# YoungWook0533/dyros_robot_controller

Hardware: AMD Instinct MI355X
Metric: QP-IK solves/s (FR3 7-DoF, batch 65k) + achieved HBM GB/s vs peak (higher is better)
Workload: dtype f64; 1 GPU; FR3 QPIKStep (exact: certified OSQP polish), 65536 instances per GPU; robot=fr3, batch_per_gpu=65536, global_batch=65536, solver=exact, parallelism=dp1 (instances sharded, no data-path collective), task_stage=wave-per-instance

## Files before the change

### dyros_robot_controller_amd/csrc/api.cpp

```cpp
#include <hip/hip_runtime.h>

#include <chrono>
#include <cmath>
#include <cstdlib>
#include <cstddef>
#include <cstdio>
#include <cstring>
#include <memory>
#include <mutex>
#include <string>
#include <algorithm>
#include <vector>

#include "../../include/drc_amd.h"
#include "../../include/drc_amd_debug.h"
#include "dynamics.hpp"
#include "kernel_common.hpp"
#include "launch.hpp"
#include "mesh.hpp"

namespace drc_amd {

struct StreamCtx {
  hipStream_t stream = nullptr;
  hipEvent_t done = nullptr;
  uint64_t last_use = 0;
  void* pool = nullptr;
  int64_t pool_bytes = 0;
  static constexpr int kSlotInts = 32;
  static constexpr int kQueueSlotQpid = 16, kQueueSlotCf = 17, kQueueInts = 18 * kSlotInts;
  int* d_queue = nullptr;
  int* dyn_list = nullptr;
  int64_t dyn_list_cap = 0;
  void* roll = nullptr;
  int64_t roll_bytes = 0;
};
constexpr size_t kMaxStreamCtx = 8;

struct Lanes {
  std::vector<hipStream_t> lanes;
  std::vector<hipEvent_t> joins;
  std::vector<hipStream_t> sides;
  std::vector<hipEvent_t> side_fork, side_join;
  hipEvent_t fork = nullptr;
};

struct drc_model_impl {
  HostModel hm;
  DevModel* d_model = nullptr;
  double* d_mesh = nullptr;
  int device = 0;
  drc_kinematic_param kparam{};
  drc_joint_index jidx{};
  drc_actuator_index aidx{};
  std::vector<std::unique_ptr<StreamCtx>> ctxs;
  uint64_t ctx_tick = 0;
  Lanes ln;
  int timing = 0;
  int lane_stage = 0;
  int eqp_small_cap = -1;
  std::vector<std::pair<std::vector<hipEvent_t>, int>> events;
  std::vector<hipEvent_t> evpool;
  int chunks = 4;
  int fused = 1;
  int32_t* d_order = nullptr;
  int64_t order_n = 0;
  std::mutex host_mu;
  void* stage = nullptr;
  int64_t stage_bytes = 0;
  double* pinned = nullptr;
  int64_t pinned_bytes = 0;
  hipStream_t hstream = nullptr;
  hipEvent_t hdone = nullptr;
  int tl_on = 0;
  std::vector<int64_t> tl;
  std::mutex mu;
  std::mutex launch_mu;
};

static thread_local std::string g_last_error;
static int set_err(int code, const std::string& msg) {
  g_last_error = msg;
  return code;
}
#define HIP_TRY(expr)                                                                   \
  do {                                                                                  \
    hipError_t e_ = (expr);                                                             \
    if (e_ != hipSuccess) return set_err(DRC_ERR_HIP, std::string(#expr) + ": " + hipGetErrorString(e_)); \
  } while (0)

static void free_ctx(StreamCtx* c) {
  if (c->done) (void)hipEventSynchronize(c->done), (void)hipEventDestroy(c->done);
  c->done = nullptr;
  if (c->d_queue) (void)hipFree(c->d_queue);
  if (c->pool) (void)hipFree(c->pool);
  if (c->dyn_list) (void)hipFree(c->dyn_list);
  if (c->roll) (void)hipFree(c->roll);
  c->roll = nullptr;
  c->roll_bytes = 0;
  c->d_queue = nullptr;
  c->pool = nullptr;
  c->dyn_list = nullptr;
}
// ... 163 lines not shown
  const double r = p.wheel_radius;
  if (p.type == DRC_DRIVE_DIFFERENTIAL) {
    *W = 2;
    const double e[6] = {1 / r, 0, -p.base_width / (2 * r), 1 / r, 0, p.base_width / (2 * r)};
    for (int i = 0; i < 6; ++i) J[i] = e[i];
    return DRC_OK;
  }
  if (p.type == DRC_DRIVE_MECANUM) {
    const int n = p.n_wheels;
    if (n < 1 || n > kMaxWheels) return set_err(DRC_ERR_INVALID_ARGUMENT, "mecanum wheel count out of range");
    for (int i = 0; i < n; ++i) {
      const double g = p.roller_angles[i], px = p.base2wheel_positions[i][0], py = p.base2wheel_positions[i][1],
                   pt = p.base2wheel_angles[i];
      const double a0 = std::cos(pt) - std::tan(g) * std::sin(pt), a1 = std::sin(pt) + std::tan(g) * std::cos(pt);
      J[i * 3 + 0] = a0 / r;
      J[i * 3 + 1] = a1 / r;
      J[i * 3 + 2] = (-a0 * py + a1 * px) / r;
    }
    *W = n;
    return DRC_OK;
  }
  if (p.type == DRC_DRIVE_CASTER) {
    const int C = p.n_wheels;
    if (C < 1 || 2 * C > kMaxWheels) return set_err(DRC_ERR_INVALID_ARGUMENT, "caster count out of range");
    const double b = p.wheel_offset;
    for (int i = 0; i < C; ++i) {
      const double phi = wheel_pos ? wheel_pos[2 * i] : 0.0, sp = std::sin(phi), cp = std::cos(phi);
      const double px = p.base2wheel_positions[i][0], py = p.base2wheel_positions[i][1];
      double* r0 = J + (2 * i) * 3;
      double* r1 = J + (2 * i + 1) * 3;
      r0[0] = -sp / b;
      r0[1] = cp / b;
      r0[2] = (px * cp + py * sp) / b - 1;
      r1[0] = cp / r;
      r1[1] = sp / r;
      r1[2] = (px * sp - py * cp) / r;
    }
    *W = 2 * C;
    return DRC_OK;
  }
  return set_err(DRC_ERR_INVALID_ARGUMENT, "unknown drive type");
}

static const char kMeshStageMsg[] =
    "the model has collision meshes: the lane-per-instance debug stage handles sphere, cylinder and box geometry only";

static int upload(drc_model_impl* m) {
  HIP_TRY(hipSetDevice(m->device));
  if (m->hm.has_mesh()) {
    const size_t bytes = m->hm.mesh_verts.size() * sizeof(double);
    HIP_TRY(hipMalloc(&m->d_mesh, bytes));
    HIP_TRY(hipMemcpy(m->d_mesh, m->hm.mesh_verts.data(), bytes, hipMemcpyHostToDevice));
    m->hm.dev.mesh_verts = m->d_mesh;
  }
  HIP_TRY(hipMalloc(&m->d_model, sizeof(DevModel)));
  HIP_TRY(hipMemcpy(m->d_model, &m->hm.dev, sizeof(DevModel), hipMemcpyHostToDevice));
  return DRC_OK;
}

static int plan_layout(const DevModel& M, KParams* k, bool task_only) {
  int off = 0;
  auto take = [&](int n) {
    int o = off;
    off += (n + 1) & ~1;
    return o;
  };
  const int nx = k->nx, ng = k->ng, np = k->np, m = k->m, nv = M.nv;
  if (task_only) {
    k->oRed = take(64);
    k->oSc = take(32);
  } else {
  k->oP = take(np * np);
  k->oG = take(ng * nx);
  k->oQ = take(nx);
  k->oAB = take(nx);
  k->oL = take(m);
  k->oU = take(m);
  k->oD = take(nx);
  k->oE = take(m);
  k->oDi = take(nx);
  k->oEi = take(m);
  k->oRho = take(m);
  k->oX = take(nx);
  k->oZ = take(m);
  k->oY = take(m);
  k->oDY = take(m);
  k->oXT = take(nx);
  k->oZT = take(m);
  k->oT1 = take(m > nx ? m : nx);
  k->oT2 = take(m > nx ? m : nx);
  k->oRed = take(64);
  k->oSc = take(32);
  k->oBc = take(nx + ng > 32 ? nx + ng : 32);
  }
  k->oHi = -1;
  if (!task_only && k->problem == 0 && M.kind == 1 && qp_compiled(nx, ng, np)) k->oHi = take(nx * nx);
  k->oU0 = off;
  if (!task_only && k->problem == 0) {
    int u = k->oU0;
    auto takeu = [&](int n) {
      int o = u;
      u += (n + 1) & ~1;
      return o;
    };
    k->kq = takeu(nv);
    k->kJ = takeu(6 * nv);
// ... 876 lines not shown
  const int virtual_dof = 3;
  d.kind = 1;
  d.n_wheel = W;
  d.n_arm = d.nv - (virtual_dof + W);
  d.virtual_start = ji->virtual_start;
  d.mani_start = ji->mani_start;
  d.mobi_start = ji->mobi_start;
  d.act_mani_start = ai->mani_start;
  d.act_mobi_start = ai->mobi_start;
  d.dyn_origin = ji->virtual_start + 3;
  if (d.n_arm < 1 || d.n_arm > 8 || ji->virtual_start + 3 > d.nv || ji->mani_start + d.n_arm > d.nv ||
      ji->mobi_start + W > d.nv || ai->mani_start + d.n_arm > d.n_arm + W || ai->mobi_start + W > d.n_arm + W) {
    delete m;
    return drc_amd::set_err(DRC_ERR_INVALID_ARGUMENT, "JointIndex/ActuatorIndex inconsistent with the URDF dof");
  }
  m->kparam = *param;
  m->jidx = *ji;
  m->aidx = *ai;
  m->device = device;
  rc = drc_amd::upload(m);
  if (rc) {
    delete m;
    return rc;
  }
  *out = m;
  return DRC_OK;
}

int drc_model_release_stream(drc_model* m, void* stream) {
  using drc_amd::set_err;
  if (!m) return drc_amd::set_err(DRC_ERR_INVALID_ARGUMENT, "null model");
  std::lock_guard<std::mutex> launch_lock(m->launch_mu);
  std::lock_guard<std::mutex> g(m->mu);
  HIP_TRY(hipSetDevice(m->device));
  hipStream_t st = reinterpret_cast<hipStream_t>(stream);
  for (size_t i = 0; i < m->ctxs.size(); ++i)
    if (m->ctxs[i]->stream == st) {
      HIP_TRY(hipStreamSynchronize(st));
      drc_amd::free_ctx(m->ctxs[i].get());
      m->ctxs.erase(m->ctxs.begin() + static_cast<std::ptrdiff_t>(i));
      break;
    }
  return DRC_OK;
}

void drc_model_destroy(drc_model* m) {
  if (!m) return;
  (void)hipSetDevice(m->device);
  (void)hipDeviceSynchronize();
  for (auto& c : m->ctxs) drc_amd::free_ctx(c.get());
  drc_amd::free_lanes(&m->ln);
  if (m->d_model) (void)hipFree(m->d_model);
  if (m->d_mesh) (void)hipFree(m->d_mesh);
  if (m->d_order) (void)hipFree(m->d_order);
  if (m->hstream) (void)hipStreamSynchronize(m->hstream), (void)hipStreamDestroy(m->hstream);
  if (m->stage) (void)hipFree(m->stage);
  if (m->pinned) (void)hipHostFree(m->pinned);
  if (m->hdone) (void)hipEventDestroy(m->hdone);
  for (auto& evs : m->events) {
    std::vector<hipEvent_t> u = evs.first;
    std::sort(u.begin(), u.end());
    u.erase(std::unique(u.begin(), u.end()), u.end());
    for (hipEvent_t e : u) (void)hipEventDestroy(e);
  }
  for (hipEvent_t e : m->evpool) (void)hipEventDestroy(e);
  delete m;
}

int drc_model_info(const drc_model* m, int* dof, int* act, int* mani, int* mobi, int* ngeom, int* npairs) {
  if (!m) return drc_amd::set_err(DRC_ERR_INVALID_ARGUMENT, "null model");
  const drc_amd::DevModel& d = m->hm.dev;
  if (dof) *dof = d.nv;
  if (act) *act = d.kind == 1 ? d.n_arm + d.n_wheel : d.nv;
  if (mani) *mani = d.kind == 1 ? d.n_arm : d.nv;
  if (mobi) *mobi = d.kind == 1 ? d.n_wheel : 0;
  if (ngeom) *ngeom = d.ngeom;
  if (npairs) *npairs = d.npairs;
  return DRC_OK;
}

int drc_model_geom_info(const drc_model* m, int geom, int* type, double param[3], int* n_vertices,
                        double* hull_residual) {
  if (!m) return drc_amd::set_err(DRC_ERR_INVALID_ARGUMENT, "null model");
  const drc_amd::DevModel& d = m->hm.dev;
  if (geom < 0 || geom >= d.ngeom) return drc_amd::set_err(DRC_ERR_INVALID_ARGUMENT, "geometry index out of range");
  if (type) *type = d.gtype[geom];
  if (param)
    for (int i = 0; i < 3; ++i) param[i] = d.gparam[geom][i];
  if (n_vertices) *n_vertices = m->hm.mesh_count[geom];
  if (hull_residual) *hull_residual = m->hm.mesh_residual[geom];
  return DRC_OK;
}

int drc_mesh_convex_hull(const char* path, const double scale[3], int max_vertices, double* verts_out, int cap,
                         int* n_out, double* residual_out) {
  if (!path || !n_out) return drc_amd::set_err(DRC_ERR_INVALID_ARGUMENT, "null argument");
  *n_out = 0;
  drc_amd::MeshHull hull;
  std::string err;
  const int rc = drc_amd::mesh_convex_hull(path, scale, max_vertices > 0 ? max_vertices : drc_amd::kMaxMeshVerts,
                                           &hull, &err);
  if (rc) return drc_amd::set_err(rc, err);
  const int n = static_cast<int>(hull.verts.size());
  *n_out = n;
  if (residual_out) *residual_out = hull.residual;
  if (n > cap || (n > 0 && !verts_out))
// ... 728 lines not shown
```

### dyros_robot_controller_amd/csrc/model.cpp

```cpp
#include "model.hpp"

#include <algorithm>
#include <cmath>
#include <cstdio>
#include <cstring>
#include <fstream>
#include <map>
#include <memory>
#include <set>
#include <sstream>

#include "../../include/drc_amd.h"
#include "mesh.hpp"

namespace drc_amd {
namespace {

struct XmlNode {
  std::string tag;
  std::map<std::string, std::string> attr;
  std::vector<std::unique_ptr<XmlNode>> kids;
  const XmlNode* child(const char* t) const {
    for (auto& k : kids)
      if (k->tag == t) return k.get();
// ... 434 lines not shown
        *err = "SRDF: " + e2;
        return DRC_ERR_PARSE;
      }
      std::set<std::pair<int, int>> drop;
      for (const XmlNode* d : sr->children("disable_collisions")) {
        const char* l1 = d->get("link1");
        const char* l2 = d->get("link2");
        if (!l1 || !l2 || !b.frame_of_link.count(l1) || !b.frame_of_link.count(l2)) continue;
        if (std::string(l1) == l2) continue;
        for (int a = 0; a < m.ngeom; ++a) {
          if (b.geom_link[a] != l1) continue;
          for (int c = 0; c < m.ngeom; ++c)
            if (b.geom_link[c] == l2) drop.insert({std::min(a, c), std::max(a, c)});
        }
      }
      std::vector<std::pair<int, int>> kept;
      for (auto& p : pairs)
        if (!drop.count(p)) kept.push_back(p);
      pairs.swap(kept);
    }
  }
  if (static_cast<int>(pairs.size()) > kMaxPairs) {
    *err = "too many collision pairs";
    return DRC_ERR_UNSUPPORTED;
  }
  m.npairs = static_cast<int>(pairs.size());
  for (int p = 0; p < m.npairs; ++p) {
    m.pair_a[p] = static_cast<int16_t>(pairs[p].first);
    m.pair_b[p] = static_cast<int16_t>(pairs[p].second);
  }
  {
    int n = 0;
    for (int cls = 0; cls < 7; ++cls)
      for (int p = 0; p < m.npairs; ++p) {
        int ta = m.gtype[m.pair_a[p]], tb = m.gtype[m.pair_b[p]];
        if (ta > tb) std::swap(ta, tb);
        const int c = tb == kMesh ? 6 : (ta == 0 ? tb : (ta == 1 ? 2 + tb : 5));
        if (c == cls) m.pair_order[n++] = static_cast<int16_t>(p);
      }
    for (int sl = 0; sl < m.npairs; ++sl) {
      m.slot_a[sl] = m.pair_a[m.pair_order[sl]];
      m.slot_b[sl] = m.pair_b[m.pair_order[sl]];
    }
  }
  m.ncand_slots = 0;
  for (int p = 0; p < m.npairs; ++p) {
    m.cand_slot[p] = -1;
    if (m.gtype[m.pair_a[p]] != kSphere && m.gtype[m.pair_b[p]] != kSphere) {
      if (m.ncand_slots < kMaxCandSlots) m.cand_pair[m.ncand_slots] = static_cast<int16_t>(p);
      m.cand_slot[p] = static_cast<int16_t>(m.ncand_slots < kMaxCandSlots ? m.ncand_slots : -1);
      ++m.ncand_slots;
    }
  }
  return DRC_OK;
}

}
```

### dyros_robot_controller_amd/csrc/model.hpp

```cpp
#pragma once

#include <cstdint>
#include <string>
#include <vector>

namespace drc_amd {

constexpr int kMaxJoints = 16;
constexpr int kMaxGeoms = 64;
constexpr int kMaxPairs = 1024;
constexpr int kMaxFrames = 64;
constexpr int kMaxWheels = 8;
constexpr int kMaxCandSlots = 128;

enum JointType : int { kRevolute = 0, kPrismatic = 1 };
enum GeomType : int { kSphere = 0, kCylinder = 1, kBox = 2, kMesh = 3 };
enum DriveKind : int { kDriveDifferential = 0, kDriveMecanum = 1, kDriveCaster = 2 };

struct DevModel {
  int nv, ngeom, npairs, nframes;
  int kind;
  int n_arm, n_wheel;
  int virtual_start, mani_start, mobi_start;
  int act_mani_start, act_mobi_start;
  int parent[kMaxJoints + 1];
  int jtype[kMaxJoints + 1];
  uint32_t anc[kMaxJoints + 1];
  double jplace[kMaxJoints + 1][12];
  double axis[kMaxJoints + 1][3];
  double lower[kMaxJoints], upper[kMaxJoints], vel[kMaxJoints];
  int frame_joint[kMaxFrames];
  double frame_place[kMaxFrames][12];
  int gparent[kMaxGeoms];
  int gtype[kMaxGeoms];
  double gplace[kMaxGeoms][12];
  double gparam[kMaxGeoms][3];
  double gbound[kMaxGeoms];
  int16_t pair_a[kMaxPairs], pair_b[kMaxPairs];
  int16_t cand_slot[kMaxPairs];
  int16_t cand_pair[kMaxCandSlots];
  int ncand_slots;
  int16_t pair_order[kMaxPairs];
  int16_t slot_a[kMaxPairs], slot_b[kMaxPairs];
  double J_mobile[3][kMaxWheels];
  int drive;
  double wheel_radius, wheel_offset;
  double caster_pos[kMaxWheels / 2][2];
  double inertia[kMaxJoints + 1][10];
  int dyn_origin;
  int has_mesh;
  int gmesh_first[kMaxGeoms], gmesh_count[kMaxGeoms];
  const double* mesh_verts;
};

struct HostModel {
  DevModel dev{};
  std::vector<std::string> joint_names;
  std::vector<std::string> frame_names;
  std::vector<std::string> geom_names;
  std::vector<double> effort;
  std::vector<double> mesh_verts;
  std::vector<int> mesh_first, mesh_count;
  std::vector<double> mesh_residual;
  std::vector<std::string> mesh_files;
  bool has_mesh() const { return !mesh_verts.empty(); }
};

int build_model_from_urdf(const std::string& urdf_path, const std::string& srdf_path,
                          const std::string& packages_path, HostModel* out, std::string* err);

}
```

### dyros_robot_controller_amd/csrc/task_stage.hpp

```cpp
#pragma once

#include "kernel_common.hpp"

namespace drc_amd {

__device__ __forceinline__ void col_dot(const DevModel* M, const double* T, const double* Zw, const double* qd, int nv,
                                        int c, V3 p, V3 pdot, uint32_t mask, V3* lin, V3* ang) {
  const V3 oc = v3(T[12 * c + 9], T[12 * c + 10], T[12 * c + 11]), zc = ld3(Zw + 3 * c);
  V3 w = v3(0, 0, 0), od = v3(0, 0, 0);
  const uint32_t ac = M->anc[c] & mask;
  for (int a = 1; a <= nv; ++a) {
    if (!(ac & (1u << (a - 1)))) continue;
    const V3 za = ld3(Zw + 3 * a);
    if (M->jtype[a] == kRevolute) {
      if (a != c) w = w + qd[a - 1] * za;
      od = od + qd[a - 1] * cross(za, oc - v3(T[12 * a + 9], T[12 * a + 10], T[12 * a + 11]));
    } else {
      od = od + qd[a - 1] * za;
    }
  }
  const V3 zd = cross(w, zc);
  if (M->jtype[c] == kRevolute) {
    *lin = cross(zd, p - oc) + cross(zc, pdot - od);
    *ang = zd;
// ... 256 lines not shown
      for (int c = 0; c < nv; ++c) s += J[l * nv + c] * nu[c];
      vec[l] = xdd[l] - s;
    }
    wsync();
    if (l < nv) {
      double s = nu[l];
      for (int i = 0; i < 6; ++i) s += W[i * nv + l] * vec[i];
      out = s;
    }
  } else {
    for (int e = l; e < 6 * nv; e += 64) {
      const int i = e / nv, c = e % nv;
      double s = 0;
      for (int a = 0; a < nv; ++a) s += J[i * nv + a] * Mi[a * nv + c];
      W[e] = s;
    }
    wsync();
    if (l < 36) {
      const int a = l / 6, b = l % 6;
      double s = 0;
      for (int c = 0; c < nv; ++c) s += W[a * nv + c] * J[b * nv + c];
      A6[l] = s;
    }
    wsync();
    if (!inv6_certified(A6, Ai)) pinv_cod6_wave(A6, Ai, ws);
    for (int e = l; e < 6 * nv; e += 64) {
      const int i = e / nv, c = e % nv;
      double s = 0;
      for (int j = 0; j < 6; ++j) s += Ai[i * 6 + j] * W[j * nv + c];
      W2[e] = s;
    }
    if (l < 6) {
      double s = 0;
      for (int j = 0; j < 6; ++j) s += Ai[l * 6 + j] * xdd[j];
      vec[l] = s;
    }
    wsync();
    if (l < 6) {
      double s = 0;
      for (int c = 0; c < nv; ++c) s += W2[l * nv + c] * nu[c];
      vec[6 + l] = vec[l] - s;
    }
    wsync();
    if (l < nv) {
      double s = gv[l] + nu[l];
      for (int i = 0; i < 6; ++i) s += J[i * nv + l] * vec[6 + i];
      out = s;
    }
  }
  if (l < nv) io.out[(int64_t)l * LD + gb] = out;
  wsync();
}

template <int PROBLEM, bool MESH = false>
__device__ __forceinline__ void task_instance(const DevModel* __restrict__ M0, const KParams& kp, const IO& io, double* S,
                                              int64_t b) {
  const int l = lane_id();
  const int nv = kp.nv;
  EpaPoly* ews = reinterpret_cast<EpaPoly*>(S + kp.kEpa);
  PH_DECL
  const int64_t gb = io.b0 + b, LD = io.ld;
  PH_ONLY(const unsigned long long inst_t0 = __builtin_amdgcn_s_memtime(); unsigned long long ph_snap[8];
          for (int k_ = 0; k_ < 8; ++k_) ph_snap[k_] = ph_acc[k_];
          unsigned long long epa_calls = 0, epa_steps = 0, epa_maxsteps = 0, epa_t[8] = {0, 0, 0, 0, 0, 0, 0, 0};)
  const DevModel* M = opaque_model(M0);
  double* qv = S + kp.kq;
  double* qd = S + kp.kqd;
  if (l < nv) {
    qv[l] = io.q[l * LD + gb];
    qd[l] = io.qdot[l * LD + gb];
  }
  double tgt = 0.0;
  if (PROBLEM == 2 && kp.cf == 3) {
  } else if (l < 12) {
    if (kp.mode != DRC_MODE_QPIK) tgt = io.xt[l * LD + gb];
  } else if (l < 18) {
    tgt = io.xdt[(l - 12) * LD + gb];
  } else if (l < 36 && kp.mode == DRC_MODE_QPIK_CUBIC) {
    tgt = l < 30 ? io.xi[(l - 18) * LD + gb] : io.xdi[(l - 30) * LD + gb];
  }
  wsync();
  double* T = S + kp.kT;
  double* Zw = S + kp.kZ;
  if (l < 12) T[l] = (l == 0 || l == 4 || l == 8) ? 1.0 : 0.0;
  double* loc = S + kp.kTg;
  if (l >= 1 && l <= nv) {
    const int j = l;
    double Mj[12];
    const double* ax = M->axis[j];
    const double qq = qv[j - 1];
    if (M->jtype[j] == kRevolute) {
      double c = cos(qq), s = sin(qq), C = 1 - c, x = ax[0], y = ax[1], z = ax[2];
      Mj[0] = c + x * x * C; Mj[1] = x * y * C - z * s; Mj[2] = x * z * C + y * s;
      Mj[3] = y * x * C + z * s; Mj[4] = c + y * y * C; Mj[5] = y * z * C - x * s;
      Mj[6] = z * x * C - y * s; Mj[7] = z * y * C + x * s; Mj[8] = c + z * z * C;
      Mj[9] = Mj[10] = Mj[11] = 0;
    } else {
      Mj[0] = Mj[4] = Mj[8] = 1;
      Mj[1] = Mj[2] = Mj[3] = Mj[5] = Mj[6] = Mj[7] = 0;
      Mj[9] = ax[0] * qq; Mj[10] = ax[1] * qq; Mj[11] = ax[2] * qq;
    }
    double Lj[12];
    tmul(M->jplace[j], Mj, Lj);
    for (int i = 0; i < 12; ++i) loc[(j - 1) * 12 + i] = Lj[i];
  }
  wsync();
  for (int j = 1; j <= nv; ++j) {
    const double* a = T + M->parent[j] * 12;
    const double* bb = loc + (j - 1) * 12;
    double v = 0;
    if (l < 9) {
      int r = l / 3, c = l % 3;
      v = a[3 * r] * bb[c] + a[3 * r + 1] * bb[3 + c] + a[3 * r + 2] * bb[6 + c];
    } else if (l < 12) {
      int r = l - 9;
      v = a[3 * r] * bb[9] + a[3 * r + 1] * bb[10] + a[3 * r + 2] * bb[11] + a[9 + r];
    }
    wsync();
    if (l < 12) T[j * 12 + l] = v;
    wsync();
  }
  double* Te = S + kp.kTe;
  if (l >= 1 && l <= nv) st3(Zw + 3 * l, rot(T + 12 * l, ld3(M->axis[l])));
  if (l == 0) tmul(T + 12 * kp.frame_joint, kp.frame_place, Te);
  wsync();
  double* Tg = S + kp.kTg;
  for (int g = l; g < M->ngeom; g += 64) {
    double out[12];
    tmul(T + 12 * M->gparent[g], M->gplace[g], out);
    for (int i = 0; i < 12; ++i) Tg[g * 12 + i] = out[i];
  }
  PH(0);
  double* J = S + kp.kJ;
  const V3 pe = v3(Te[9], Te[10], Te[11]);
  const uint32_t anc_e = M->anc[kp.frame_joint];
  if (l < nv) {
    const int j = l + 1;
    V3 lin = v3(0, 0, 0), ang = v3(0, 0, 0);
    if (anc_e & (1u << l)) {
      V3 z = ld3(Zw + 3 * j);
      if (M->jtype[j] == kRevolute) {
        lin = cross(z, pe - v3(T[12 * j + 9], T[12 * j + 10], T[12 * j + 11]));
        ang = z;
      } else {
        lin = z;
      }
    }
    J[0 * nv + l] = lin.x; J[1 * nv + l] = lin.y; J[2 * nv + l] = lin.z;
    J[3 * nv + l] = ang.x; J[4 * nv + l] = ang.y; J[5 * nv + l] = ang.z;
  }
  wsync();
  double* xdd = S + kp.kxdd;
  double jq = 0.0;
  if (l < 6)
    for (int c = 0; c < nv; ++c) jq += J[l * nv + c] * qd[c];
  if (l == 0) {
    if (kp.mode == DRC_MODE_QPIK) {
      for (int i = 0; i < 6; ++i) xdd[i] = rd_lane(tgt, 12 + i);
    } else {
      double xt[12], xdt[6];
      for (int i = 0; i < 12; ++i) xt[i] = rd_lane(tgt, i);
      for (int i = 0; i < 6; ++i) xdt[i] = rd_lane(tgt, 12 + i);
      if (kp.mode == DRC_MODE_QPIK_CUBIC) {
        double xi[12], xdi[6], Rt[9], Ri[9];
        for (int i = 0; i < 12; ++i) xi[i] = rd_lane(tgt, 18 + i);
        for (int i = 0; i < 6; ++i) xdi[i] = rd_lane(tgt, 30 + i);
        for (int r = 0; r < 3; ++r)
          for (int c = 0; c < 3; ++c) {
            Rt[3 * r + c] = xt[3 * c + r];
            Ri[3 * r + c] = xi[3 * c + r];
          }
        const double t = kp.t, t0 = kp.t0, tf = kp.t0 + kp.duration;
        double pd[3], vd[3];
        for (int i = 0; i < 3; ++i) {
          pd[i] = cubic(t, t0, tf, xi[9 + i], xt[9 + i], xdi[i], xdt[i]);
          vd[i] = cubic_dot(t, t0, tf, xi[9 + i], xt[9 + i], xdi[i], xdt[i]);
        }
        double RiT_Rt[9], Rd[9];
        for (int a = 0; a < 3; ++a)
          for (int c = 0; c < 3; ++c)
            RiT_Rt[3 * a + c] = Ri[a] * Rt[c] + Ri[3 + a] * Rt[3 + c] + Ri[6 + a] * Rt[6 + c];
        V3 r = so3_log(RiT_Rt);
        if (t >= tf) {
          for (int i = 0; i < 9; ++i) Rd[i] = Rt[i];
        } else if (t < t0) {
          for (int i = 0; i < 9; ++i) Rd[i] = Ri[i];
        } else {
          double E3[9];
          so3_exp(cubic(t, t0, tf, 0, 1, 0, 0) * r, E3);
          for (int a = 0; a < 3; ++a)
            for (int c = 0; c < 3; ++c)
              Rd[3 * a + c] = Ri[3 * a] * E3[c] + Ri[3 * a + 1] * E3[3 + c] + Ri[3 * a + 2] * E3[6 + c];
        }
        V3 rd = v3(cubic_dot(t, t0, tf, 0, r.x, 0, 0), cubic_dot(t, t0, tf, 0, r.y, 0, 0),
// ... 42 lines not shown
    int a = l / 6, bb = l % 6;
    double s = 0;
    for (int c = 0; c < narm; ++c) s += J[a * nv + c0 + c] * J[bb * nv + c0 + c];
    A6[l] = s;
  }
  wsync();
  {
    double piv_min = 1e300, det = 1;
    const int lr = l < 6 ? l : 0;
    double r6[6];
#pragma unroll
    for (int j = 0; j < 6; ++j) r6[j] = A6[lr * 6 + j];
#pragma unroll
    for (int k = 0; k < 6; ++k) {
      const double akk = bcast(r6[k], k), aik = r6[k], ia = 1.0 / akk;
      double pk6[6];
#pragma unroll
      for (int j = 0; j < 6; ++j) pk6[j] = bcast(r6[j], k);
#pragma unroll
      for (int j = 0; j < 6; ++j) {
        double v;
        if (l == k && j == k) v = ia;
        else if (l == k) v = pk6[j] * ia;
        else if (j == k) v = -aik * ia;
        else v = r6[j] - aik * (pk6[j] * ia);
        r6[j] = v;
      }
      piv_min = fmin(piv_min, akk);
      det *= akk;
    }
    if (l < 6)
#pragma unroll
      for (int j = 0; j < 6; ++j) Ai[l * 6 + j] = r6[j];
    wsync();
    const double fa = wave_sum(l < 36 ? A6[l] * A6[l] : 0.0), fi = wave_sum(l < 36 ? Ai[l] * Ai[l] : 0.0);
    if (!(piv_min > 0) || !(fa * fi < 1e10)) {
      const double dt = det_lu6_wave(A6);
      pinv_cod6_wave(A6, Ai, S + kp.kScr);
      if (l == 0) S[kp.oSc + SC_MAN] = sqrt(dt);
    } else if (l == 0) {
      S[kp.oSc + SC_MAN] = sqrt(det);
    }
    wsync();
  }
  double* W = S + kp.kW;
  for (int e = l; e < narm * 6; e += 64) {
    int c = e / 6, a = e % 6;
    double s = 0;
    for (int i = 0; i < 6; ++i) s += J[i * nv + c0 + c] * Ai[i * 6 + a];
    W[e] = s;
  }
  wsync();
  double* part = S + kp.kPart;
  for (int e = l; e < narm * narm; e += 64) {
    const int kk = e / narm, c = e % narm;
    const int jk = c0 + kk + 1, ji = c0 + c + 1;
    double acc = 0;
    if ((anc_e & (1u << (jk - 1))) && (anc_e & (1u << (ji - 1)))) {
      V3 zk = ld3(Zw + 3 * jk), zi = ld3(Zw + 3 * ji);
      V3 pk_ = v3(T[12 * jk + 9], T[12 * jk + 10], T[12 * jk + 11]);
      V3 pi_ = v3(T[12 * ji + 9], T[12 * ji + 10], T[12 * ji + 11]);
      const bool krev = M->jtype[jk] == kRevolute;
      V3 dpe = krev ? cross(zk, pe - pk_) : zk;
      const bool moves_i = jk != ji && (M->anc[ji] & (1u << (jk - 1)));
      V3 dzi = (moves_i && krev) ? cross(zk, zi) : v3(0, 0, 0);
      V3 dpi = moves_i ? (krev ? cross(zk, pi_ - pk_) : zk) : v3(0, 0, 0);
      V3 lin, ang;
      if (M->jtype[ji] == kRevolute) {
        lin = cross(dzi, pe - pi_) + cross(zi, dpe - dpi);
        ang = dzi;
      } else {
        lin = dzi;
        ang = v3(0, 0, 0);
      }
      const double* w = W + c * 6;
      acc = lin.x * w[0] + lin.y * w[1] + lin.z * w[2] + ang.x * w[3] + ang.y * w[4] + ang.z * w[5];
    }
    part[e] = acc;
  }
  wsync();
  double* mg = S + kp.kmg;
  if (l < narm) {
    double s = 0;
    for (int c = 0; c < narm; ++c) s += part[l * narm + c];
    mg[l] = S[kp.oSc + SC_MAN] * s;
  }
  PH(2);
  double* pd = S + kp.kPd;
  int8_t* pf = reinterpret_cast<int8_t*>(S + kp.kPf);
  double bestd = 1.7976931348623157e308;
  int besti = 0x7fffffff;
  int bhow = 0;
  V3 bpA = v3(0, 0, 0), bpB = v3(0, 0, 0);
  double ub = 1e300;
  [[maybe_unused]] auto hull_shape = [&](int g) {
    return ShapeMT<lds_pose*, true>{M->gtype[g], (lds_pose*)(Tg + 12 * g), M->gparam[g][0], M->gparam[g][1],
                                    M->gparam[g][2], M->mesh_verts + 3 * M->gmesh_first[g], M->gmesh_count[g]};
  };
  for (int sl = l; sl < M->npairs; sl += 64) {
    const int p = M->pair_order[sl], ga = M->slot_a[sl], gb = M->slot_b[sl];
    ShapeL A{M->gtype[ga], (lds_pose*)(Tg + 12 * ga), M->gparam[ga][0], M->gparam[ga][1], M->gparam[ga][2]};
    ShapeL Bs{M->gtype[gb], (lds_pose*)(Tg + 12 * gb), M->gparam[gb][0], M->gparam[gb][1], M->gparam[gb][2]};
    V3 pA, pB;
    double d;
    if constexpr (MESH) {
      if (A.type == kMesh || Bs.type == kMesh) {
        if (A.type == kMesh) A.type = kBox;
        if (Bs.type == kMesh) Bs.type = kBox;
        pd[p] = (A.type == kSphere || Bs.type == kSphere) ? sphere_pair(A, Bs, &pA, &pB)
                                                          : pair_lower_bound(A, Bs, M->gbound[ga], M->gbound[gb]);
        pf[p] = 0;
        continue;
      }
    }
    const bool closed = (A.type == kSphere || Bs.type == kSphere)
                            ? (d = sphere_pair(A, Bs, &pA, &pB), true)
                            : (A.type == kCylinder && Bs.type == kCylinder && cyl_cyl_side(A, Bs, &d, &pA, &pB));
    if (closed) {
      pf[p] = 1;
      ub = fmin(ub, d);
      if (d < bestd || (d == bestd && p < besti)) {
        bestd = d;
        besti = p;
        bhow = 0;
        bpA = pA;
        bpB = pB;
      }
    } else {
      pd[p] = pair_lower_bound(A, Bs, M->gbound[ga], M->gbound[gb]);
      pf[p] = 0;
    }
  }
  ub = -wave_max(-ub);
  PH(3);
  bool pen = false;
  {
    int* cand = reinterpret_cast<int*>(S + kp.kCand);
    int ncand = 0;
    [[maybe_unused]] int nhull = 0;
    for (int p0 = 0; p0 < M->npairs; p0 += 64) {
      const int p = p0 + l;
      bool c = p < M->npairs && pf[p] == 0 && pd[p] - 1e-9 <= ub;
      if constexpr (MESH) {
        const bool h = c && (M->gtype[M->pair_a[p]] == kMesh || M->gtype[M->pair_b[p]] == kMesh);
        const unsigned long long mh = __ballot(h);
        if (h) cand[M->npairs - 1 - (nhull + __popcll(mh & ((1ull << l) - 1)))] = p;
        nhull += __popcll(mh);
        c = c && !h;
      }
      const unsigned long long m = __ballot(c);
      if (c) cand[ncand + __popcll(m & ((1ull << l) - 1))] = p;
      ncand += __popcll(m);
    }
    if (l == 0) ews->nv = 0;
    wsync();
    for (int c = l; c < ncand; c += 64) {
      const int p = cand[c];
      const int ga = M->pair_a[p], gb = M->pair_b[p];
      ShapeL A{M->gtype[ga], (lds_pose*)(Tg + 12 * ga), M->gparam[ga][0], M->gparam[ga][1], M->gparam[ga][2]};
      ShapeL Bs{M->gtype[gb], (lds_pose*)(Tg + 12 * gb), M->gparam[gb][0], M->gparam[gb][1], M->gparam[gb][2]};
      const GjkDist g = gjk(A, Bs, ub + 1e-9, ews, p);
      if (g.pruned) {
        pf[p] = 1;
      } else if (g.intersect) {
        pf[p] = 2;
        pen = true;
      } else {
        pf[p] = 1;
        if (g.dist < bestd || (g.dist == bestd && p < besti)) {
          bestd = g.dist;
          besti = p;
          bhow = 1;
          bpA = g.pA;
          bpB = g.pB;
        }
      }
    }
    if constexpr (MESH) {
      ub = fmin(ub, -wave_max(-bestd));
      for (int c = 0; c < nhull; ++c) {
        const int p = cand[M->npairs - 1 - c];
        const int ga = M->pair_a[p], gb = M->pair_b[p];
// ... 81 lines not shown
        bpB = ld3(ews->out + 3);
      }
      if (dall < gbd || (dall == gbd && p < gbi)) {
        gbd = dall;
        gbi = p;
      }
      if (l == ln) pf[p] = 1;
      wsync();
    }
#ifdef DRC_EPA_PRIO
    __builtin_amdgcn_s_setprio(0);
#endif
  }
  PH(5);
  const double myd = bestd;
  const int myi = besti;
  wave_argmin(bestd, besti);
  double* dgv = S + kp.kdg;
  double* red = S + kp.oRed;
  auto refine_winner = [&]() {
    const int ga = M->pair_a[besti], gb = M->pair_b[besti];
    const ShapeL A{M->gtype[ga], (lds_pose*)(Tg + 12 * ga), M->gparam[ga][0], M->gparam[ga][1], M->gparam[ga][2]};
    const ShapeL Bs{M->gtype[gb], (lds_pose*)(Tg + 12 * gb), M->gparam[gb][0], M->gparam[gb][1], M->gparam[gb][2]};
    double dref = S[kp.oSc + SC_DIST];
    V3 rA = ld3(red), rB = ld3(red + 3);
    if constexpr (MESH) {
      if (A.type == kMesh || Bs.type == kMesh) {
        if (refine_witness_hull(serial_shape(hull_shape(ga)), serial_shape(hull_shape(gb)), &dref, &rA, &rB)) {
          st3(red, rA);
          st3(red + 3, rB);
          S[kp.oSc + SC_DIST] = dref;
        }
        return;
      }
    }
#ifdef DRC_NO_REFINE
    if (false && refine_witness(A, Bs, &dref, &rA, &rB)) {
#else
    if (refine_witness(A, Bs, &dref, &rA, &rB)) {
#endif
      st3(red, rA);
      st3(red + 3, rB);
      S[kp.oSc + SC_DIST] = dref;
    }
  };
  auto dist_grad = [&](double dd) {
    double g = 0;
    if (besti < M->npairs) {
      const int jA = M->gparent[M->pair_a[besti]], jB = M->gparent[M->pair_b[besti]];
      V3 pA = ld3(red), pB = ld3(red + 3), n = pB - pA;
      n = (1.0 / sqrt(dot(n, n))) * n;
      const int j = l + 1;
      V3 z = ld3(Zw + 3 * j), pj = v3(T[12 * j + 9], T[12 * j + 10], T[12 * j + 11]);
      const bool rev = M->jtype[j] == kRevolute;
      V3 cA = v3(0, 0, 0), cB = v3(0, 0, 0);
      if (jA > 0 && (M->anc[jA] & (1u << l))) cA = rev ? cross(z, pA - pj) : z;
      if (jB > 0 && (M->anc[jB] & (1u << l))) cB = rev ? cross(z, pB - pj) : z;
      g = dot(n, cB - cA);
      if (dd < 0) g = -g;
    }
    return g;
  };
  if (myi == besti && myi < M->npairs) {
    st3(red, bpA);
    st3(red + 3, bpB);
    S[kp.oSc + SC_DIST] = myd;
    S[kp.oSc + SC_HOW] = bhow;
  }
  if (l == 0) {
    if (besti >= M->npairs) {
      S[kp.oSc + SC_DIST] = bestd;
      S[kp.oSc + SC_HOW] = 0;
    }
    S[kp.oSc + SC_PAIR] = besti;
  }
  wsync();
  if constexpr (PROBLEM == 1) {
    if (l == 0 && S[kp.oSc + SC_HOW] != 0) refine_winner();
    wsync();
  }
  bestd = S[kp.oSc + SC_DIST];
  PH(6);
  if (l < nv) dgv[l] = dist_grad(bestd);
  wsync();
  if constexpr (PROBLEM == 1) qpid_task_extras(M, kp, S, bestd, besti, io.st_gdv != nullptr);
  PH(7);
  PH_ONLY(if (l == 0) {
    const unsigned long long dt = __builtin_amdgcn_s_memtime() - inst_t0;
    atomicMax(&g_phase_cycles[30], dt);
    if (dt > 400000ull) {
      atomicAdd(&g_phase_cycles[31], 1ull);
      atomicAdd(&g_phase_cycles[29], dt);
      for (int k_ = 0; k_ < 8; ++k_) atomicAdd(&g_phase_cycles[8 + k_], ph_acc[k_] - ph_snap[k_]);
    }
    if (epa_calls) {
      atomicAdd(&g_phase_cycles[22], epa_calls);
      atomicAdd(&g_phase_cycles[23], epa_steps);
      atomicMax(&g_phase_cycles[28], epa_maxsteps);
      atomicAdd(&g_phase_cycles[18], epa_t[0] + epa_t[1]);
      atomicAdd(&g_phase_cycles[20], epa_t[2]);
      atomicAdd(&g_phase_cycles[59], epa_t[3]);
      atomicAdd(&g_phase_cycles[61], epa_t[4]);
      atomicAdd(&g_phase_cycles[62], epa_t[5]);
      atomicAdd(&g_phase_cycles[63], epa_t[6]);
      atomicAdd(&g_phase_cycles[60], epa_t[7]);
    }
  })
// ... 63 lines not shown
```

Baseline: 38.03 million solves/s.

## Precompute SoA collision pair table and joint bitmasks for task stage

Builds a host-side structure-of-arrays table of per-pair metadata, shape parameters and bounds, indexed by slot, so that each lane in the pair loop does coalesced global loads instead of gathering from DevModel arrays through index indirection. It also adds revolute and ancestor bitmasks that replace per-joint array lookups, hoists each lane's joint and geom placement loads ahead of the sync barriers, and switches to sincos. These changes target scattered model-memory gathers in the per-instance wave. The cost is an extra device allocation, and the bitmask layout assumes at most 16 joints.

Measured after the change: 39.00 million solves/s, median of 6. +2.5%, better.

```diff
diff --git a/dyros_robot_controller_amd/csrc/api.cpp b/dyros_robot_controller_amd/csrc/api.cpp
--- a/dyros_robot_controller_amd/csrc/api.cpp
+++ b/dyros_robot_controller_amd/csrc/api.cpp
@@ -49,6 +49,7 @@
   HostModel hm;
   DevModel* d_model = nullptr;
   double* d_mesh = nullptr;
+  double* d_pair_tab = nullptr;
   int device = 0;
   drc_kinematic_param kparam{};
   drc_joint_index jidx{};
@@ -318,6 +319,12 @@
     HIP_TRY(hipMalloc(&m->d_mesh, bytes));
     HIP_TRY(hipMemcpy(m->d_mesh, m->hm.mesh_verts.data(), bytes, hipMemcpyHostToDevice));
     m->hm.dev.mesh_verts = m->d_mesh;
+  }
+  {
+    const size_t bytes = m->hm.pair_tab.size() * sizeof(double);
+    HIP_TRY(hipMalloc(&m->d_pair_tab, bytes));
+    HIP_TRY(hipMemcpy(m->d_pair_tab, m->hm.pair_tab.data(), bytes, hipMemcpyHostToDevice));
+    m->hm.dev.pair_tab = m->d_pair_tab;
   }
   HIP_TRY(hipMalloc(&m->d_model, sizeof(DevModel)));
   HIP_TRY(hipMemcpy(m->d_model, &m->hm.dev, sizeof(DevModel), hipMemcpyHostToDevice));
@@ -1300,6 +1307,7 @@
   drc_amd::free_lanes(&m->ln);
   if (m->d_model) (void)hipFree(m->d_model);
   if (m->d_mesh) (void)hipFree(m->d_mesh);
+  if (m->d_pair_tab) (void)hipFree(m->d_pair_tab);
   if (m->d_order) (void)hipFree(m->d_order);
   if (m->hstream) (void)hipStreamSynchronize(m->hstream), (void)hipStreamDestroy(m->hstream);
   if (m->stage) (void)hipFree(m->stage);
diff --git a/dyros_robot_controller_amd/csrc/model.cpp b/dyros_robot_controller_amd/csrc/model.cpp
--- a/dyros_robot_controller_amd/csrc/model.cpp
+++ b/dyros_robot_controller_amd/csrc/model.cpp
@@ -510,7 +510,37 @@
       ++m.ncand_slots;
     }
   }
+  build_stage_tables(out);
   return DRC_OK;
 }
 
-}
+void build_stage_tables(HostModel* hm) {
+  DevModel& m = hm->dev;
+  m.rev_mask = 0;
+  for (int w = 0; w < 4; ++w) m.anc_bits[w] = 0;
+  for (int j = 1; j <= m.nv; ++j) {
+    if (m.jtype[j] == kRevolute) m.rev_mask |= 1u << (j - 1);
+    for (int k = 1; k <= m.nv; ++k)
+      if (m.anc[j] & (1u << (k - 1))) {
+        const int bit = 16 * (j - 1) + (k - 1);
+        m.anc_bits[bit >> 6] |= 1ull << (bit & 63);
+      }
+  }
+  m.pair_ld = (m.npairs + 63) / 64 * 64;
+  hm->pair_tab.assign(static_cast<size_t>(kPairFields) * std::max(m.pair_ld, 1), 0.0);
+  for (int sl = 0; sl < m.npairs; ++sl) {
+    const int p = m.pair_order[sl], ga = m.pair_a[p], gb = m.pair_b[p];
+    double* rec = hm->pair_tab.data() + sl;
+    const uint64_t meta = static_cast<uint64_t>(p) | static_cast<uint64_t>(ga) << 16 | static_cast<uint64_t>(gb) << 24 |
+                          static_cast<uint64_t>(m.gtype[ga]) << 32 | static_cast<uint64_t>(m.gtype[gb]) << 36;
+    std::memcpy(rec + kPairMeta * m.pair_ld, &meta, sizeof(meta));
+    for (int k = 0; k < 3; ++k) {
+      rec[(kPairParamA + k) * m.pair_ld] = m.gparam[ga][k];
+      rec[(kPairParamB + k) * m.pair_ld] = m.gparam[gb][k];
+    }
+    rec[kPairBoundA * m.pair_ld] = m.gbound[ga];
+    rec[kPairBoundB * m.pair_ld] = m.gbound[gb];
+  }
+}
+
+}
diff --git a/dyros_robot_controller_amd/csrc/model.hpp b/dyros_robot_controller_amd/csrc/model.hpp
--- a/dyros_robot_controller_amd/csrc/model.hpp
+++ b/dyros_robot_controller_amd/csrc/model.hpp
@@ -51,7 +51,13 @@
   int has_mesh;
   int gmesh_first[kMaxGeoms], gmesh_count[kMaxGeoms];
   const double* mesh_verts;
+  uint32_t rev_mask;
+  uint64_t anc_bits[4];
+  const double* pair_tab;
+  int pair_ld;
 };
+constexpr int kPairFields = 9;
+constexpr int kPairMeta = 0, kPairParamA = 1, kPairParamB = 4, kPairBoundA = 7, kPairBoundB = 8;
 
 struct HostModel {
   DevModel dev{};
@@ -63,10 +69,12 @@
   std::vector<int> mesh_first, mesh_count;
   std::vector<double> mesh_residual;
   std::vector<std::string> mesh_files;
+  std::vector<double> pair_tab;
   bool has_mesh() const { return !mesh_verts.empty(); }
 };
 
 int build_model_from_urdf(const std::string& urdf_path, const std::string& srdf_path,
                           const std::string& packages_path, HostModel* out, std::string* err);
+void build_stage_tables(HostModel* hm);
 
 }
diff --git a/dyros_robot_controller_amd/csrc/task_stage.hpp b/dyros_robot_controller_amd/csrc/task_stage.hpp
--- a/dyros_robot_controller_amd/csrc/task_stage.hpp
+++ b/dyros_robot_controller_amd/csrc/task_stage.hpp
@@ -332,6 +332,51 @@
   wsync();
 }
 
+#ifdef __HIP_DEVICE_COMPILE__
+typedef __attribute__((address_space(1))) const double glb_cdouble;
+#else
+typedef const double glb_cdouble;
+#endif
+struct PairTab {
+  glb_cdouble* t;
+  int ld;
+};
+__device__ __forceinline__ PairTab pair_tab(const DevModel* M) { return PairTab{(glb_cdouble*)M->pair_tab, M->pair_ld}; }
+struct PairRec {
+  int p, ga, gb, ta, tb;
+  double pa[3], pb[3], ba, bb;
+};
+__device__ __forceinline__ PairRec pair_rec(const PairTab& pt, int i) {
+  glb_cdouble* t = pt.t + i;
+  PairRec r;
+  const unsigned long long m = static_cast<unsigned long long>(__double_as_longlong(t[kPairMeta * pt.ld]));
+#pragma unroll
+  for (int k = 0; k < 3; ++k) {
+    r.pa[k] = t[(kPairParamA + k) * pt.ld];
+    r.pb[k] = t[(kPairParamB + k) * pt.ld];
+  }
+  r.ba = t[kPairBoundA * pt.ld];
+  r.bb = t[kPairBoundB * pt.ld];
+  r.p = static_cast<int>(m & 0xffffu);
+  r.ga = static_cast<int>((m >> 16) & 0xffu);
+  r.gb = static_cast<int>((m >> 24) & 0xffu);
+  r.ta = static_cast<int>((m >> 32) & 0xfu);
+  r.tb = static_cast<int>((m >> 36) & 0xfu);
+  return r;
+}
+struct AncBits {
+  uint64_t w[4];
+};
+__device__ __forceinline__ AncBits anc_bits(const DevModel* M) {
+  return AncBits{{M->anc_bits[0], M->anc_bits[1], M->anc_bits[2], M->anc_bits[3]}};
+}
+__device__ __forceinline__ bool supports(const AncBits& ab, int k, int j) {
+  const int bit = 16 * (j - 1) + (k - 1), w = bit >> 6;
+  const uint64_t x = w == 0 ? ab.w[0] : (w == 1 ? ab.w[1] : (w == 2 ? ab.w[2] : ab.w[3]));
+  return (x >> (bit & 63)) & 1u;
+}
+__device__ __forceinline__ bool revolute(uint32_t rev_mask, int j) { return (rev_mask >> (j - 1)) & 1u; }
+
 template <int PROBLEM, bool MESH = false>
 __device__ __forceinline__ void task_instance(const DevModel* __restrict__ M0, const KParams& kp, const IO& io, double* S,
                                               int64_t b) {
@@ -350,6 +395,12 @@
     qv[l] = io.q[l * LD + gb];
     qd[l] = io.qdot[l * LD + gb];
   }
+  const uint32_t rev_mask = M->rev_mask;
+  const int jm = l <= nv ? l : 0, gm = l < M->ngeom ? l : 0;
+  double jpl[12];
+#pragma unroll
+  for (int i = 0; i < 12; ++i) jpl[i] = M->jplace[jm][i];
+  const V3 axl = ld3(M->axis[jm]);
   double tgt = 0.0;
   if (PROBLEM == 2 && kp.cf == 3) {
   } else if (l < 12) {
@@ -367,10 +418,12 @@
   if (l >= 1 && l <= nv) {
     const int j = l;
     double Mj[12];
-    const double* ax = M->axis[j];
+    const double ax[3] = {axl.x, axl.y, axl.z};
     const double qq = qv[j - 1];
-    if (M->jtype[j] == kRevolute) {
-      double c = cos(qq), s = sin(qq), C = 1 - c, x = ax[0], y = ax[1], z = ax[2];
+    if (revolute(rev_mask, j)) {
+      double c, s;
+      sincos(qq, &s, &c);
+      double C = 1 - c, x = ax[0], y = ax[1], z = ax[2];
       Mj[0] = c + x * x * C; Mj[1] = x * y * C - z * s; Mj[2] = x * z * C + y * s;
       Mj[3] = y * x * C + z * s; Mj[4] = c + y * y * C; Mj[5] = y * z * C - x * s;
       Mj[6] = z * x * C - y * s; Mj[7] = z * y * C + x * s; Mj[8] = c + z * z * C;
@@ -381,10 +434,14 @@
       Mj[9] = ax[0] * qq; Mj[10] = ax[1] * qq; Mj[11] = ax[2] * qq;
     }
     double Lj[12];
-    tmul(M->jplace[j], Mj, Lj);
+    tmul(jpl, Mj, Lj);
     for (int i = 0; i < 12; ++i) loc[(j - 1) * 12 + i] = Lj[i];
   }
   wsync();
+  double gpl[12];
+#pragma unroll
+  for (int i = 0; i < 12; ++i) gpl[i] = M->gplace[gm][i];
+  const int gpar = M->gparent[gm];
   for (int j = 1; j <= nv; ++j) {
     const double* a = T + M->parent[j] * 12;
     const double* bb = loc + (j - 1) * 12;
@@ -401,14 +458,14 @@
     wsync();
   }
   double* Te = S + kp.kTe;
-  if (l >= 1 && l <= nv) st3(Zw + 3 * l, rot(T + 12 * l, ld3(M->axis[l])));
+  if (l >= 1 && l <= nv) st3(Zw + 3 * l, rot(T + 12 * l, axl));
   if (l == 0) tmul(T + 12 * kp.frame_joint, kp.frame_place, Te);
   wsync();
   double* Tg = S + kp.kTg;
-  for (int g = l; g < M->ngeom; g += 64) {
+  if (l < M->ngeom) {
     double out[12];
-    tmul(T + 12 * M->gparent[g], M->gplace[g], out);
-    for (int i = 0; i < 12; ++i) Tg[g * 12 + i] = out[i];
+    tmul(T + 12 * gpar, gpl, out);
+    for (int i = 0; i < 12; ++i) Tg[l * 12 + i] = out[i];
   }
   PH(0);
   double* J = S + kp.kJ;
@@ -419,7 +476,7 @@
     V3 lin = v3(0, 0, 0), ang = v3(0, 0, 0);
     if (anc_e & (1u << l)) {
       V3 z = ld3(Zw + 3 * j);
-      if (M->jtype[j] == kRevolute) {
+      if (revolute(rev_mask, j)) {
         lin = cross(z, pe - v3(T[12 * j + 9], T[12 * j + 10], T[12 * j + 11]));
         ang = z;
       } else {
@@ -568,6 +625,7 @@
   }
   wsync();
   double* part = S + kp.kPart;
+  const AncBits ancb = anc_bits(M);
   for (int e = l; e < narm * narm; e += 64) {
     const int kk = e / narm, c = e % narm;
     const int jk = c0 + kk + 1, ji = c0 + c + 1;
@@ -576,13 +634,13 @@
       V3 zk = ld3(Zw + 3 * jk), zi = ld3(Zw + 3 * ji);
       V3 pk_ = v3(T[12 * jk + 9], T[12 * jk + 10], T[12 * jk + 11]);
       V3 pi_ = v3(T[12 * ji + 9], T[12 * ji + 10], T[12 * ji + 11]);
-      const bool krev = M->jtype[jk] == kRevolute;
+      const bool krev = revolute(rev_mask, jk);
       V3 dpe = krev ? cross(zk, pe - pk_) : zk;
-      const bool moves_i = jk != ji && (M->anc[ji] & (1u << (jk - 1)));
+      const bool moves_i = jk != ji && supports(ancb, jk, ji);
       V3 dzi = (moves_i && krev) ? cross(zk, zi) : v3(0, 0, 0);
       V3 dpi = moves_i ? (krev ? cross(zk, pi_ - pk_) : zk) : v3(0, 0, 0);
       V3 lin, ang;
-      if (M->jtype[ji] == kRevolute) {
+      if (revolute(rev_mask, ji)) {
         lin = cross(dzi, pe - pi_) + cross(zi, dpe - dpi);
         ang = dzi;
       } else {
@@ -613,10 +671,12 @@
     return ShapeMT<lds_pose*, true>{M->gtype[g], (lds_pose*)(Tg + 12 * g), M->gparam[g][0], M->gparam[g][1],
                                     M->gparam[g][2], M->mesh_verts + 3 * M->gmesh_first[g], M->gmesh_count[g]};
   };
+  const PairTab ptab = pair_tab(M);
   for (int sl = l; sl < M->npairs; sl += 64) {
-    const int p = M->pair_order[sl], ga = M->slot_a[sl], gb = M->slot_b[sl];
-    ShapeL A{M->gtype[ga], (lds_pose*)(Tg + 12 * ga), M->gparam[ga][0], M->gparam[ga][1], M->gparam[ga][2]};
-    ShapeL Bs{M->gtype[gb], (lds_pose*)(Tg + 12 * gb), M->gparam[gb][0], M->gparam[gb][1], M->gparam[gb][2]};
+    const PairRec pr = pair_rec(ptab, sl);
+    const int p = pr.p;
+    ShapeL A{pr.ta, (lds_pose*)(Tg + 12 * pr.ga), pr.pa[0], pr.pa[1], pr.pa[2]};
+    ShapeL Bs{pr.tb, (lds_pose*)(Tg + 12 * pr.gb), pr.pb[0], pr.pb[1], pr.pb[2]};
     V3 pA, pB;
     double d;
     if constexpr (MESH) {
@@ -624,7 +684,7 @@
         if (A.type == kMesh) A.type = kBox;
         if (Bs.type == kMesh) Bs.type = kBox;
         pd[p] = (A.type == kSphere || Bs.type == kSphere) ? sphere_pair(A, Bs, &pA, &pB)
-                                                          : pair_lower_bound(A, Bs, M->gbound[ga], M->gbound[gb]);
+                                                          : pair_lower_bound(A, Bs, pr.ba, pr.bb);
         pf[p] = 0;
         continue;
       }
@@ -643,7 +703,7 @@
         bpB = pB;
       }
     } else {
-      pd[p] = pair_lower_bound(A, Bs, M->gbound[ga], M->gbound[gb]);
+      pd[p] = pair_lower_bound(A, Bs, pr.ba, pr.bb);
       pf[p] = 0;
     }
   }
@@ -831,7 +891,7 @@
       n = (1.0 / sqrt(dot(n, n))) * n;
       const int j = l + 1;
       V3 z = ld3(Zw + 3 * j), pj = v3(T[12 * j + 9], T[12 * j + 10], T[12 * j + 11]);
-      const bool rev = M->jtype[j] == kRevolute;
+      const bool rev = revolute(rev_mask, j);
       V3 cA = v3(0, 0, 0), cB = v3(0, 0, 0);
       if (jA > 0 && (M->anc[jA] & (1u << l))) cA = rev ? cross(z, pA - pj) : z;
       if (jB > 0 && (M->anc[jB] & (1u << l))) cB = rev ? cross(z, pB - pj) : z;
```
